# vovach777/llcomp

Hardware: AMD Instinct MI355X
Metric: encode+decode MPix/s on 4K RGB8, bit-exact (higher is better)
Workload: dtype int32

## Files before the change

llcomp_amd/csrc/codec.hip:

```cpp
#include <hip/hip_runtime.h>

#include <algorithm>
#include <cstdlib>
#include <cstring>
#include <mutex>
#include <new>
#include <vector>

#include "../../include/llcomp_mi.h"
#include "codec_internal.hpp"
#include "container.hpp"
#include "geometry.hpp"
#include "kernels.hpp"
#include "resize.hpp"
#include "snapshot.hpp"
#include "tables.hpp"
#include "update.hpp"

using namespace llcomp_mi;

namespace llcomp_mi {

int status_from_bits(uint32_t bits) {
    if (bits & kStInternal) return LLCOMP_MI_HIP_ERROR;
// ... 571 lines not shown
                 uint64_t* d_total, uint32_t* d_status, hipStream_t s) {
    Timed t(k, s, 3);
    if (!encoder_writes_group_sums(g)) HIP_TRY(launch_group_sums(g, d_slice_len, d_group_off, s));
    HIP_TRY(launch_scan_groups(g, d_group_off, d_total, s));
    HIP_TRY(launch_pack_payload(g, k->d_scratch, d_slice_len, d_group_off, d_payload, payload_cap, d_status, s));
    return LLCOMP_MI_OK;
}

}

namespace llcomp_mi {
void codec_release(llcomp_mi_codec* k) {
    if (!k) return;
    DeviceGuard guard(k->device);
    if (k->done && k->done->ev && hipEventQuery(k->done->ev) != hipErrorNotReady) {
        (void)hipGetLastError();
        k->done.reset();
    }
    dev_free(k->d_sym_or_rec, k->done);
    dev_free(k->d_lane_order, k->done);
    dev_free(k->d_states, k->done);
    dev_free(k->d_scratch, k->done);
    dev_free(k->d_group_off, k->done);
    dev_free(k->d_total_tmp, k->done);
    dev_free(k->d_region_len, k->done);
    dev_free(k->d_region_off, k->done);
    dev_free(k->d_regions, k->done);
    dev_free(k->d_stage, k->done);
    dev_free(k->d_box, k->done);
    dev_free(k->d_mid, k->done);
    dev_free(k->d_upd_goff, k->done);
    for (uint32_t i = 0; i < llcomp_mi_codec::kRegionsRing; ++i) {
        if (!k->h_regions[i]) continue;
        if (k->regions_ev_live[i] && k->regions_ev[i] && hipEventQuery(k->regions_ev[i]) == hipErrorNotReady) (void)hipEventSynchronize(k->regions_ev[i]);
        (void)hipGetLastError();
        (void)hipHostFree(k->h_regions[i]);
    }
    for (auto& ev : k->regions_ev) if (ev) (void)hipEventDestroy(ev);
    dev_free(k->d_snap_sorted, k->done);
    dev_free(k->d_snap_banks, k->done);
    dev_free(k->d_snap_res, k->done);
    dev_free(k->d_snap_ctx, k->done);
    dev_free(k->d_snap_io, k->done);
    dev_free(k->d_seg_state, k->done);
    if (k->ev_fork) (void)hipEventDestroy(k->ev_fork);
    for (auto& ev : k->ev_chunk) if (ev) (void)hipEventDestroy(ev);
// ... 74 lines not shown
    if (!guard.ok) return LLCOMP_MI_HIP_ERROR;
    llcomp_mi_codec* k = new (std::nothrow) llcomp_mi_codec;
    if (!k) return LLCOMP_MI_NOMEM;
    k->g = g;
    k->tune = current_tuning();
    k->device = dev;
    k->feedback = !current_tuning().nofeedback;
    k->overlap = current_tuning().overlap != 0;
    k->aux_shared = current_tuning().overlap == 2;
    const uint64_t samples = uint64_t(frames) * w * h * c;
    k->need_states = slices_need_state_tables(g);
    const bool fused = model_is_fused(g);
    const uint64_t b_sym = fused ? 8 : samples * 4, b_states = k->need_states ? (uint64_t(lane_groups(g)) * kContexts << g.lane_shift) * 8 : 8,
                   b_scratch = (uint64_t(lane_groups(g)) << g.lane_shift) * g.slice_cap, b_off = (uint64_t(lane_groups(g)) + 1) * 8;
    const bool snap = snapshot_mode(g);
    const uint64_t snap_el = snap ? snapshot_elems(g) : 0;
    const uint64_t b_lanes = std::max((uint64_t(lane_groups(g)) * slice_capacity_samples(g) << g.lane_shift) * (fused ? 2 : 4), snap_el * 4);
    const uint64_t b_region = uint64_t(g.n_slices) * 12 +
                              (!k->need_states && !rows_mode(g) ? (uint64_t(lane_groups(g)) * kContexts << g.lane_shift) * 8 : 0);
    const uint64_t b_regions = uint64_t(frames) * sizeof(RegionsFrame) + stage_bound(g);
    const uint64_t b_resized = 2 * samples + resized_tables_bound(g);
    const uint64_t b_update = (uint64_t(g.n_slices) + 1 + lane_groups(g) + 1) * 8 +
                              (snap ? 0 : region_snapshot_bound(g) ? region_snapshot_bound(g) * 28 + uint64_t(g.n_slices) * 64 : 0);
    k->workspace_bytes = b_sym + b_lanes + b_states + b_scratch + b_off + 8 + snap_el * (snapshot_chunked(g) ? 28 : 18) + b_region + b_regions +
                         b_resized + b_update;
    const bool ok = dev_alloc(&k->d_sym_or_rec, b_sym) == hipSuccess && dev_alloc(&k->d_lane_order, b_lanes) == hipSuccess &&
                    dev_alloc(reinterpret_cast<void**>(&k->d_scratch), b_scratch) == hipSuccess &&
                    dev_alloc(reinterpret_cast<void**>(&k->d_group_off), b_off) == hipSuccess &&
                    dev_alloc(reinterpret_cast<void**>(&k->d_total_tmp), 8) == hipSuccess &&
                    dev_alloc(reinterpret_cast<void**>(&k->d_counters), kCtrCount * 8) == hipSuccess &&
                    hipMemset(k->d_counters, 0, kCtrCount * 8) == hipSuccess;
    if (!ok) {
        llcomp_mi_codec_destroy(k);
        return LLCOMP_MI_NOMEM;
    }
    k->allocated_bytes = b_sym + b_lanes + b_scratch + b_off + 8;
    *out = k;
    return LLCOMP_MI_OK;
}

extern "C" {

void llcomp_mi_codec_destroy(llcomp_mi_codec* k) {
    llcomp_mi::codec_release(k);
}

int llcomp_mi_codec_prepare(llcomp_mi_codec* k, uint32_t what) {
    if (!k || (what & ~(LLCOMP_MI_PREPARE_ENCODE | LLCOMP_MI_PREPARE_DECODE | LLCOMP_MI_PREPARE_REGION | LLCOMP_MI_PREPARE_REGIONS |
                        LLCOMP_MI_PREPARE_RESIZED | LLCOMP_MI_PREPARE_UPDATE)))
        return LLCOMP_MI_BAD_ARGS;
    DeviceGuard guard(k->device);
    if (!guard.ok) return LLCOMP_MI_HIP_ERROR;
    if (what & LLCOMP_MI_PREPARE_ENCODE) {
        if (snapshot_mode(k->g)) {
            if (int rc = ensure_snapshot_arrays(k, k->g)) return rc;
        }
        if (!snapshot_mode(k->g) || snapshot_chunked(k->g))
            if (int rc = ensure_state_tables(k, k->need_states)) return rc;
    }
// ... 60 lines not shown
    if (!guard.ok) return LLCOMP_MI_HIP_ERROR;
    hipStream_t s = static_cast<hipStream_t>(stream);
    const Geometry& g = k->g;
    DoneGuard done_guard{k, s};
    HIP_TRY(hipMemsetAsync(d_status, 0, 4, s));
    {
        Timed t(k, s, 7);
        if (int rc = next_state_generation(k, s, k->need_states)) return rc;
    }
    {
        Timed t(k, s, 4);
        HIP_TRY(launch_group_sums(g, static_cast<const uint32_t*>(d_slice_len), k->d_group_off, s));
        HIP_TRY(launch_scan_groups(g, k->d_group_off, k->d_total_tmp, s));
    }
    {
        Timed t(k, s, 4);
        HIP_TRY(launch_stage_streams(g, static_cast<const uint8_t*>(d_payload), payload_bytes,
                                     static_cast<const uint32_t*>(d_slice_len), k->d_group_off, k->d_scratch,
                                     static_cast<uint32_t*>(d_status), s));
    }
    {
        Timed t(k, s, 5);
        const bool cache = use_bank_cache(k, g);
        HIP_TRY(launch_decode_slices(g, k->d_scratch, static_cast<const uint32_t*>(d_slice_len), k->d_states, k->state_generation,
                                     static_cast<int16_t*>(k->d_lane_order), static_cast<uint32_t*>(d_status), k->d_counters, cache, s));
        if (cache) queue_feedback(k, s);
    }
    {
        Timed t(k, s, 6);
        if (model_is_fused(g)) {
            HIP_TRY(launch_model_rows_inv(g, static_cast<const int16_t*>(k->d_lane_order), static_cast<uint8_t*>(d_px), s));
        } else {
            HIP_TRY(launch_from_lane_order_i16(g, static_cast<const int16_t*>(k->d_lane_order),
                                               static_cast<int16_t*>(k->d_sym_or_rec), s));
            HIP_TRY(launch_model_inv(g, static_cast<const int16_t*>(k->d_sym_or_rec), static_cast<uint8_t*>(d_px), s));
        }
    }
    ++k->n_decode;
    return LLCOMP_MI_OK;
}

uint32_t llcomp_mi_codec_region_family(const llcomp_mi_codec* k, uint32_t x, uint32_t y, uint32_t rw, uint32_t rh) {
    RegionBox box;
    Geometry sub;
    if (!k || region_setup(k, x, y, rw, rh, box, sub)) return 0;
    return (sub.flags & 0xFFu) | (sub.lane_shift << 8) | (sub.lpw << 16);
}

int llcomp_mi_codec_decode_region(llcomp_mi_codec* k, const void* d_payload, uint64_t payload_bytes, const void* d_slice_len, uint32_t x,
                                  uint32_t y, uint32_t rw, uint32_t rh, void* d_px, void* d_status, void* stream) {
    if (!k || !d_payload || !d_slice_len || !d_px || !d_status) return LLCOMP_MI_BAD_ARGS;
    RegionBox box;
    Geometry sub;
    if (int rc = region_setup(k, x, y, rw, rh, box, sub)) return rc;
// ... 440 lines not shown
```

llcomp_amd/csrc/codec_internal.hpp:

```cpp
#pragma once
#include <hip/hip_runtime.h>

#include <cstdint>
#include <memory>
#include <vector>

#include "../../include/llcomp_mi.h"
#include "geometry.hpp"
#include "kernels.hpp"

namespace llcomp_mi {
struct DoneEvent {
    hipEvent_t ev = nullptr;
    ~DoneEvent();
};
std::shared_ptr<DoneEvent> make_done_event();
}

struct llcomp_mi_codec {
    llcomp_mi::Geometry g{};
    int device = 0;
    void* d_sym_or_rec = nullptr;
    void* d_lane_order = nullptr;
    uint64_t* d_states = nullptr;
    uint8_t* d_scratch = nullptr;
    uint64_t* d_group_off = nullptr;
    uint64_t* d_total_tmp = nullptr;
    uint32_t* d_region_len = nullptr;
    uint64_t* d_region_off = nullptr;
    llcomp_mi::Tuning tune{};
    static constexpr uint32_t kRegionsRing = 4;
    llcomp_mi::RegionsFrame* d_regions = nullptr;
    uint8_t* h_regions[kRegionsRing] = {};
    uint64_t h_regions_cap[kRegionsRing] = {};
    hipEvent_t regions_ev[kRegionsRing] = {};
    bool regions_ev_live[kRegionsRing] = {};
    uint32_t regions_slot = 0;
    uint8_t* d_stage = nullptr;
    uint64_t stage_cap = 0;
    uint8_t* d_box = nullptr;
    uint64_t box_cap = 0;
    uint8_t* d_mid = nullptr;
    uint64_t mid_cap = 0;
    uint64_t* d_upd_goff = nullptr;
    uint64_t snap_el = 0;
    void* d_snap_sorted = nullptr;
    void* d_snap_banks = nullptr;
    void* d_snap_res = nullptr;
    void* d_snap_ctx = nullptr;
    void* d_snap_io = nullptr;
// ... 107 lines not shown
```

llcomp_amd/csrc/geometry.hpp:

```cpp
#pragma once
#include <algorithm>
#include <cstdint>
#include <cstdlib>

#if defined(__HIPCC__)
#define LLMI_HD __host__ __device__
#else
#define LLMI_HD
#endif

namespace llcomp_mi {

constexpr uint32_t kMaxChannels = 255;

struct Geometry {
    uint32_t frames, w, h, c;
    uint32_t tile_w, tile_h, planar;
    uint32_t ntx, nty;
    uint32_t slices_per_frame;
    uint32_t n_slices;
    uint32_t slice_cap;
    uint32_t nch;
    uint32_t lane_shift;
    uint32_t slice_samples;
    uint32_t lpw;
    uint32_t flags;
};
enum : uint32_t {
    kGeoRows = 1u,
    kGeoLdsTable = 2u,
    kGeoForceReplay = 4u,
    kGeoSmallModel = 8u,
    kGeoSnapshot = 16u,
    kGeoBankCache = 32u,
};
constexpr uint32_t kSnapMaxSamples = 4096;
constexpr uint32_t kSnapMaxChunks = 4;

struct Tuning {
    int lane_shift = -1;
    int lpw = 0;
    bool norows = false;
    bool noldstab = false;
    bool force_replay = false;
    bool nosnap = false;
    bool nocache = false;
    int overlap = 2;
    bool nofeedback = false;
};
inline Tuning tuning_from_env() {
    Tuning t;
    auto num = [](const char* name, long lo, long hi, int dflt) {
        const char* e = std::getenv(name);
        if (!e || !*e) return dflt;
        const long v = std::strtol(e, nullptr, 10);
        return (v >= lo && v <= hi) ? int(v) : dflt;
    };
    auto flag = [](const char* name) { const char* e = std::getenv(name); return e && e[0] == '1'; };
    t.lane_shift = num("LLCOMP_MI_LANE_SHIFT", 0, 6, -1);
    t.lpw = num("LLCOMP_MI_LPW", 1, 64, 0);
    t.norows = flag("LLCOMP_MI_NOROWS");
    t.noldstab = flag("LLCOMP_MI_NOLDSTAB");
    t.force_replay = flag("LLCOMP_MI_FORCE_REPLAY");
    t.nosnap = flag("LLCOMP_MI_NOSNAP");
    t.nocache = flag("LLCOMP_MI_NOCACHE");
    t.nofeedback = flag("LLCOMP_MI_NOFEEDBACK");
    t.overlap = num("LLCOMP_MI_OVERLAP", 0, 2, 2);
    return t;
}

LLMI_HD inline uint32_t snapshot_chunks(const Geometry& g) { return (g.slice_samples + kSnapMaxSamples - 1) / kSnapMaxSamples; }
LLMI_HD inline uint32_t snapshot_cap(const Geometry& g) {
    return g.slice_samples <= kSnapMaxSamples ? (g.slice_samples + 15u) & ~15u : snapshot_chunks(g) * kSnapMaxSamples;
}

constexpr int kBankCacheLog2 = 5;
inline int bank_cache_log2(const Geometry& g) { return (g.flags & kGeoBankCache) ? kBankCacheLog2 : 0; }

LLMI_HD inline uint32_t rows_px_dwords(uint64_t tile_base, uint32_t samples, uint32_t c, uint64_t batch_bytes) {
    if (tile_base + 4 > batch_bytes) return 0;
    const uint64_t k = (batch_bytes - 4 - tile_base) / c + 1;
    return k < samples ? uint32_t(k) : samples;
}
LLMI_HD inline uint32_t rows_px_tail(uint32_t c) { return 1 + (4 + c - 1) / c; }

LLMI_HD inline size_t lane_order_index(const Geometry& g, uint32_t id, uint32_t k) {
    const uint32_t gw = 1u << g.lane_shift;
    return ((size_t(id >> g.lane_shift) * g.slice_samples + k) << g.lane_shift) + (id & (gw - 1));
// ... 199 lines not shown
```

llcomp_amd/csrc/kernels.hpp:

```cpp
#pragma once
#include <hip/hip_runtime.h>

#include <cstdint>

#include "geometry.hpp"

namespace llcomp_mi {

enum : uint32_t { kStOverflow = 1u, kStBadExponent = 2u, kStTruncated = 4u, kStInternal = 8u  };

enum : uint32_t {
    kCtrDecCachedWaves = 0,
    kCtrDecBypassedWaves = 1,
    kCtrCacheLookups = 2,
    kCtrCacheMisses = 3,
    kCtrCacheWritebacks = 4,
    kCtrDecReplays = 5,
    kCtrEncCarryBacks = 6,
    kCtrGenerationWraps = 7,
    kCtrDecLaunchesCached = 8,
    kCtrDecLaunchesPlainByFeedback = 9,
    kCtrCount = 16,
};

// ... 16 lines not shown
hipError_t launch_encode_slices(const Geometry& g, const void* d_sym, uint64_t* d_states, uint32_t generation, uint8_t* d_scratch,
                                uint32_t* d_slice_len, uint64_t* d_group_off, uint32_t* d_status, unsigned long long* d_counters,
                                hipStream_t stream);
uint64_t state_generation_tag(uint32_t generation);
hipError_t launch_encode_segment(const Geometry& g, const void* d_res, uint64_t* d_banks, uint8_t* d_scratch, uint32_t* d_slice_len,
                                 uint32_t* d_status, unsigned long long* d_counters, uint32_t seg_first, uint32_t* d_seg_state,
                                 hipStream_t stream);
bool encoder_writes_group_sums(const Geometry& g);
hipError_t launch_group_sums(const Geometry& g, const uint32_t* d_slice_len, uint64_t* d_group_off, hipStream_t stream);
hipError_t launch_scan_groups(const Geometry& g, uint64_t* d_group_off, uint64_t* d_total, hipStream_t stream);
hipError_t launch_frame_bytes(const Geometry& g, const uint32_t* d_slice_len, uint64_t* d_frame_bytes, hipStream_t stream);
hipError_t launch_pack_payload(const Geometry& g, const uint8_t* d_units, const uint32_t* d_slice_len,
                               const uint64_t* d_group_off, uint8_t* d_payload, uint64_t payload_cap,
                               uint32_t* d_status, hipStream_t stream);
hipError_t launch_stage_streams(const Geometry& g, const uint8_t* d_payload, uint64_t payload_bytes,
                                const uint32_t* d_slice_len, const uint64_t* d_group_off, uint8_t* d_units,
                                uint32_t* d_status, hipStream_t stream);
hipError_t launch_copy_segments(const uint8_t* d_src, uint8_t* d_dst, const uint64_t* d_src_off, const uint64_t* d_dst_off,
                                const uint64_t* d_len, uint32_t n_seg, uint64_t max_len, hipStream_t stream);
hipError_t launch_range_sums(const uint32_t* d_vals, const uint64_t* d_start, const uint64_t* d_count, uint64_t* d_out, uint32_t n,
                             uint32_t cap, hipStream_t stream);
hipError_t launch_decode_slices(const Geometry& g, const uint8_t* d_units, const uint32_t* d_slice_len,
                                uint64_t* d_states, uint32_t generation, int16_t* d_rec, uint32_t* d_status, unsigned long long* d_counters,
                                bool bank_cache, hipStream_t stream);

hipError_t launch_region_index(const Geometry& full, const Geometry& sub, const RegionBox& box, const uint32_t* d_slice_len,
                               const uint64_t* d_group_off, uint32_t* d_sub_len, uint64_t* d_sub_off, hipStream_t stream);
hipError_t launch_stage_region_streams(const Geometry& sub, const uint8_t* d_payload, uint64_t payload_bytes, const uint32_t* d_sub_len,
                                       const uint64_t* d_sub_off, uint8_t* d_units, uint32_t* d_status, hipStream_t stream);
struct Crop {
    uint32_t x0, y0, rw, rh;
};
hipError_t launch_model_inv_crop(const Geometry& sub, const int16_t* d_rec, uint8_t* d_px, const Crop& cr, hipStream_t stream);
hipError_t launch_model_rows_inv_crop(const Geometry& sub, const int16_t* d_lanes, uint8_t* d_px, const Crop& cr, hipStream_t stream);

hipError_t launch_regions_index(const Geometry& full, const Geometry& sub, const RegionsFrame* d_tab, const uint32_t* d_slice_len,
                                const uint64_t* d_group_off, uint32_t* d_sub_len, uint64_t* d_sub_off, hipStream_t stream);
hipError_t launch_model_inv_crops(const Geometry& sub, const int16_t* d_rec, uint8_t* d_px, const RegionsFrame* d_tab, uint32_t rw,
                                  uint32_t rh, hipStream_t stream);
hipError_t launch_model_rows_inv_crops(const Geometry& sub, const int16_t* d_lanes, uint8_t* d_px, const RegionsFrame* d_tab, uint32_t rw,
                                       uint32_t rh, hipStream_t stream);

}
```

llcomp_amd/csrc/model_kernels.hip:

```cpp
#include <algorithm>

#include "device_common.hpp"
#include "kernels.hpp"

namespace llcomp_mi {

namespace {

constexpr int kMW = 256;
constexpr int kMH = 32;

template <int C>
__device__ __forceinline__ void rct_forward(const uint8_t* p, int16_t (&o)[C]) {
    if constexpr (C >= 3) {
        const int g = p[1], cb = int(p[2]) - g, cr = int(p[0]) - g;
        o[0] = int16_t(cr);
        o[1] = int16_t(g + (cb + cr) / 4);
        o[2] = int16_t(cb);
        if constexpr (C == 4) o[3] = p[3];
    } else {
#pragma unroll
        for (int k = 0; k < C; ++k) o[k] = p[k];
    }
}

template <int C>
// ... 583 lines not shown
__host__ inline uint64_t xcd_grid(uint32_t n_groups, uint32_t chunks) { return uint64_t((n_groups + kXcds - 1) / kXcds) * kXcds * chunks; }
__device__ __forceinline__ bool xcd_chunk_group(uint32_t n_groups, uint32_t chunks, uint32_t& group, uint32_t& chunk) {
    const uint32_t xcd = blockIdx.x % kXcds, slot = blockIdx.x / kXcds;
    const uint32_t per_class = (chunks + kXcds - 1) / kXcds;
    group = slot / per_class;
    chunk = xcd + kXcds * (slot - group * per_class);
    return group < n_groups && chunk < chunks;
}
__host__ inline uint64_t xcd_chunk_grid(uint32_t n_groups, uint32_t chunks) { return uint64_t(n_groups) * ((chunks + kXcds - 1) / kXcds) * kXcds; }

template <int C>
__device__ __forceinline__ void rct_pixel(const uint8_t* p, int (&v)[C]) {
    if constexpr (C >= 3) {
        const int g = p[1], cb = int(p[2]) - g, cr = int(p[0]) - g;
        v[0] = cr;
        v[1] = g + (cb + cr) / 4;
        v[2] = cb;
        if constexpr (C == 4) v[3] = p[3];
    } else {
#pragma unroll
        for (int k = 0; k < C; ++k) v[k] = p[k];
    }
}
struct RowTile {
    unsigned long long base;
    uint32_t sw;
};
template <int C>
__device__ __forceinline__ void load_row_tiles(const Geometry& g, uint32_t first_tile, uint32_t ntiles, RowTile* tiles) {
    if (threadIdx.x < ntiles) {
        const uint32_t tile = first_tile + threadIdx.x;
        const uint32_t per_frame = g.ntx * g.nty;
        const uint32_t frame = tile / per_frame, rem = tile - frame * per_frame;
        const uint32_t y = rem / g.ntx, tx = rem - y * g.ntx;
        const uint32_t x0 = tx * g.tile_w;
        tiles[threadIdx.x].base = ((size_t(frame) * g.h + y) * g.w + x0) * C;
        tiles[threadIdx.x].sw = g.w - x0 < g.tile_w ? g.w - x0 : g.tile_w;
    }
}

typedef short s16x2 __attribute__((ext_vector_type(2)));
typedef unsigned short u16x2 __attribute__((ext_vector_type(2)));
__device__ __forceinline__ u16x2 pk_min_u16(u16x2 a, u16x2 b) {
    u16x2 d;
    asm("v_pk_min_u16 %0, %1, %2" : "=v"(d) : "v"(a), "v"(b));
    return d;
}

template <int C>
__global__ __launch_bounds__(256) void k_model_rows_fwd(const Geometry g, const uint8_t* __restrict__ px,
                                                        uint16_t* __restrict__ lanes) {
    constexpr int K = 64, RUN = (K + 2) * C, TPG = 64 / C + 2;
    constexpr int RUNW = (RUN + 3) / 4 + 1;
    constexpr int PADL = (C - 1 + 1) & ~1, OCOLS = (PADL + 64 + C - 1 + 1) & ~1;
    __shared__ uint32_t raw[TPG][RUNW + 1];
    __shared__ __attribute__((aligned(4))) uint16_t otile[K][OCOLS];
    __shared__ RowTile tiles[TPG];
    const uint32_t chunks = (g.tile_w + K - 1) / K;
    uint32_t group, chunk;
    if (!xcd_group_chunk((g.n_slices + (1u << g.lane_shift) - 1) >> g.lane_shift, chunks, group, chunk)) return;
    const uint32_t k0 = chunk * K;
    const uint32_t gw = 1u << g.lane_shift;
// ... 143 lines not shown
            *reinterpret_cast<uint32_t*>(&tile[kk][2 * d]) = w[it];
        }
    }
    if (g.lane_shift != 6) {
        __syncthreads();
        for (uint32_t i = threadIdx.x; i < uint32_t(K) * gw; i += 256) {
            const uint32_t kk = i / gw, col = i - kk * gw, k = k0 + kk;
            tile[kk][col] = (first_id + col < g.n_slices && k < g.tile_w) ? lanes[lane_order_index(g, first_id + col, k)] : int16_t(0);
        }
    }
    if constexpr (C > 1) {
        for (uint32_t i = threadIdx.x; i < uint32_t(K) * (C - 1); i += 256) {
            const uint32_t kk = i / (C - 1), e = i - kk * (C - 1), k = k0 + kk;
            const uint32_t id = first_id + gw + e;
            tile[kk][gw + e] = (id < g.n_slices && k < g.tile_w) ? lanes[lane_order_index(g, id, k)] : int16_t(0);
        }
    }
    __syncthreads();
    const uint32_t col0 = first_tile * C - first_id;
    const uint32_t q4 = threadIdx.x & 15;
    for (uint32_t tt = threadIdx.x >> 4; tt < ntiles; tt += 16) {
        const uint32_t sw = tiles[tt].sw, kb = k0 + 4 * q4;
        if (kb >= sw) continue;
        uint8_t bytes[4 * C];
#pragma unroll
        for (int i = 0; i < 4; ++i) {
            const int16_t* s = &tile[4 * q4 + i][col0 + tt * C];
            if constexpr (C >= 3) {
                int r = s[0], gg = s[1], bb = s[2];
                gg -= (r + bb) / 4;
                r += gg;
                bb += gg;
                bytes[i * C + 0] = uint8_t(min(max(r, 0), 255));
                bytes[i * C + 1] = uint8_t(min(max(gg, 0), 255));
                bytes[i * C + 2] = uint8_t(min(max(bb, 0), 255));
                if constexpr (C == 4) bytes[i * C + 3] = uint8_t(s[3]);
            } else {
#pragma unroll
                for (int c = 0; c < C; ++c) bytes[i * C + c] = uint8_t(s[c]);
            }
        }
        uint8_t* o = px + tiles[tt].base + size_t(kb) * C;
        const uint32_t npx = sw - kb < 4 ? sw - kb : 4;
        if (npx == 4) {
            uint32_t w[C];
#pragma unroll
            for (int c = 0; c < C; ++c)
                w[c] = uint32_t(bytes[4 * c]) | (uint32_t(bytes[4 * c + 1]) << 8) | (uint32_t(bytes[4 * c + 2]) << 16) |
                       (uint32_t(bytes[4 * c + 3]) << 24);
            __builtin_memcpy(o, w, 4 * C);
        } else {
            for (uint32_t i = 0; i < npx * C; ++i) o[i] = bytes[i];
        }
    }
}

struct RowTileCrop {
    long long base;
    uint32_t klo, khi;
};
template <int C>
__device__ __forceinline__ void load_row_tiles_crop(const Geometry& g, uint32_t first_tile, uint32_t ntiles, const Crop& cr,
                                                    RowTileCrop* tiles) {
    if (threadIdx.x < ntiles) {
        const uint32_t tile = first_tile + threadIdx.x;
        const uint32_t per_frame = g.ntx * g.nty;
        const uint32_t frame = tile / per_frame, rem = tile - frame * per_frame;
        const uint32_t y = rem / g.ntx, tx = rem - y * g.ntx;
        const uint32_t x0 = tx * g.tile_w;
        const uint32_t sw = g.w - x0 < g.tile_w ? g.w - x0 : g.tile_w;
        const uint32_t klo = cr.x0 > x0 ? cr.x0 - x0 : 0u;
        uint32_t khi = cr.x0 + cr.rw > x0 ? min(sw, cr.x0 + cr.rw - x0) : 0u;
        if (y < cr.y0 || y >= cr.y0 + cr.rh || khi <= klo) khi = 0;
        tiles[threadIdx.x].base = ((long long)(size_t(frame) * cr.rh + (y - cr.y0)) * cr.rw + (long long)x0 - (long long)cr.x0) * C;
        tiles[threadIdx.x].klo = klo;
        tiles[threadIdx.x].khi = khi;
// ... 425 lines not shown
```

llcomp_amd/csrc/slice_kernels.hip:

```cpp
#include <algorithm>

#include "device_common.hpp"
#include "kernels.hpp"

#ifndef LLMI_ASM_ENC
#define LLMI_ASM_ENC 1
#endif
#if LLMI_ASM_ENC
#include "enc_rows_asm.hpp"
#endif
#ifndef LLMI_ASM_DEC
#define LLMI_ASM_DEC 1
#endif
#if LLMI_ASM_DEC
#include "dec_rows_asm.hpp"
#endif

namespace llcomp_mi {

namespace {

#ifdef LLMI_CLOCK_PROBE
constexpr uint32_t kProbeSlots = 1u << 15;
__device__ unsigned long long g_probe[2][kProbeSlots][2];
struct ProbeStamp {
    unsigned long long t, r;
// ... 866 lines not shown
    } else
#endif
    {
        ok = hot ? dec_residual<true, false, INLDS>(d, bank, tab, v) : dec_residual<false, false, INLDS>(d, bank, tab, v);
        hot = 2 * __popcll(__ballot(v != 0)) >= __popcll(__ballot(true));
    }
    const bool ran_dry = (INLDS && LLMI_ASM_DEC != 0) ? false : d.win == 0;
    if (__builtin_expect(!ok || ran_dry || replay_always, 0)) {
        ++d.replays;
        d.low = s_low; d.range = s_range; d.win = s_win;
        bank.w[0] = s_b0; bank.w[1] = s_b1;
        if constexpr (INLDS) {
            bank.w[2] = s_b2; bank.w[3] = s_b3;
            reinterpret_cast<uint32_t*>(bank.lds)[0] = s_b0;
            reinterpret_cast<uint32_t*>(bank.lds)[64] = s_b1;
            reinterpret_cast<uint32_t*>(bank.lds)[128] = s_b2;
            reinterpret_cast<uint32_t*>(bank.lds)[192] = s_b3;
        }
        ok = dec_residual<false, true, INLDS>(d, bank, tab, v);
    }
    return ok;
}

constexpr uint32_t bank_cache_lds_bytes(int log2_entries) { return log2_entries ? (64u * 9u) << log2_entries : 0u; }
template <int NCH, bool ROWS, bool LDSTAB = false, int CACHE = 0>
__global__ __launch_bounds__(64) void k_decode_slices(const Geometry g, const uint32_t lpw_and_flags,
                                                      const uint8_t* __restrict__ units,
                                                      const uint32_t* __restrict__ slice_len,
                                                      uint64_t* __restrict__ states, int16_t* __restrict__ rec,
                                                      uint32_t* status, const uint64_t gpat,
                                                      unsigned long long* __restrict__ counters) {
    __shared__ entry_t tab[128];
    __shared__ uint32_t rowbank[ROWS ? kWideBankWords : 1];
    __shared__ int8_t quant_lut[ROWS ? 1 : 512];
    if constexpr (!ROWS) {
        for (uint32_t i = threadIdx.x; i < 256; i += blockDim.x) {
            quant_lut[i] = int8_t(quant11(int(i) - 128));
            quant_lut[256 + i] = int8_t(quant5(int(i) - 128));
        }
    }
    static_assert(CACHE == 0 || (!ROWS && !LDSTAB && NCH != 0), "the bank cache belongs to the 2-D kernels with tables in HBM");
    static_assert(CACHE == 0 || ((kContexts - 1) >> CACHE) < 0xFF, "bank cache: a context's tag would alias the empty marker");
    __shared__ uint32_t wave_sums[CACHE != 0 ? 2 : 1];
    clear_lds_states<LDSTAB>();
    if constexpr (CACHE != 0) {
        uint32_t* tg = reinterpret_cast<uint32_t*>(dyn_lds + (512u << CACHE));
        for (uint32_t i = threadIdx.x; i < (16u << CACHE); i += blockDim.x) tg[i] = 0xFFFFFFFFu;
        if (threadIdx.x < 2) wave_sums[threadIdx.x] = 0;
    }
    load_table(tab);
    const uint32_t lpw = lpw_and_flags & 0xFF;
    const bool replay_always = (lpw_and_flags >> 8) & 1;
    const bool small_model = (g.flags & kGeoSmallModel) != 0;
    const uint32_t id = blockIdx.x * lpw + threadIdx.x;
    if (threadIdx.x >= lpw || id >= g.n_slices) return;
    const SliceRect r = slice_rect(g, id);
    RangeDec d;
    const uint32_t len = min(slice_len[id], g.slice_cap - 16);
    const uint32_t grp = __builtin_amdgcn_readfirstlane(id >> g.lane_shift);
    const uint32_t lane_in_group = id & ((1u << g.lane_shift) - 1);
    dec_open(d, reinterpret_cast<const uint32_t*>(units) + ((size_t(grp) * (g.slice_cap >> 2)) << g.lane_shift), lane_in_group,
             g.lane_shift, len);

    int16_t* p0 = rec + lane_order_index(g, id, 0);
    const ptrdiff_t GW = ptrdiff_t(1) << g.lane_shift;
    int16_t* const gbase = rec + ((size_t(grp) * g.slice_samples) << g.lane_shift);
    uint32_t hot = 0;
    LLMI_PROBE_START();

    if constexpr (ROWS) {
        for (uint32_t k = 0; k < 12; ++k) rowbank[k * 64 + threadIdx.x] = lds_address(tab) * 0x00010001u;
        int l[NCH], L[NCH];
#pragma unroll
        for (int k = 0; k < NCH; ++k) l[k] = L[k] = 128;
        int held_val = 0;
        uint32_t held_ofs = lane_in_group * 2, next_ofs = held_ofs, step_ofs = 2u << g.lane_shift;
        uint32_t large = small_model ? 0u : ~0u, first = ~0u;
        asm volatile("" : "+v"(large), "+v"(first), "+v"(step_ofs));
        uint8_t* const bank0 = reinterpret_cast<uint8_t*>(rowbank) + threadIdx.x * 4;
        bool bad = false;
        auto pixel = [&]() {
// ... 10 lines not shown
                asm volatile("" : "+v"(o1), "+v"(o2));
                uint32_t* bp = reinterpret_cast<uint32_t*>(bank0 + (o1 + o2));
                Bank bank{{bp[0], bp[64], bp[128], bp[192]}, reinterpret_cast<uint8_t*>(bp)};
                uint32_t v = 0;
                if (!dec_sample<true>(d, bank, tab, hot, replay_always, v)) bad = true;
                v = (v ^ uint32_t(sg)) - uint32_t(sg);
                const int val = int(int16_t(uint32_t(lv) + v));
                held_val = val;
                held_ofs = next_ofs;
                next_ofs += step_ofs;
                L[k] = lv ^ ((lv ^ val) & int(first));
                l[k] = val;
            }
            first = 0;
        };
        const uint32_t sw0 = __builtin_amdgcn_readfirstlane(r.sw);
        const uint32_t n_bulk = __builtin_amdgcn_ballot_w64(r.sw != sw0) == 0 ? sw0 : 0;
        uint32_t x = 0;
        for (; x < n_bulk; ++x) pixel();
        for (; x < r.sw; ++x) pixel();
        if (bad) atomicOr(status, kStBadExponent);
        asm volatile("global_store_short %0, %1, %2" : : "v"(held_ofs), "v"(held_val), "s"(gbase) : "memory");
        publish_count(counters, kCtrDecReplays, d.replays);
    } else {
        uint64_t* banks;
        uint32_t bsh;
        if constexpr (LDSTAB) {
            banks = reinterpret_cast<uint64_t*>(dyn_lds);
            bsh = 0;
        } else {
            banks = states + ((size_t(id >> g.lane_shift) * kContexts) << g.lane_shift) + (id & ((1u << g.lane_shift) - 1));
            bsh = g.lane_shift;
        }
        if constexpr (NCH == 0) {
            const uint32_t nch = g.nch;
            const ptrdiff_t px_step = ptrdiff_t(nch) * GW, up = ptrdiff_t(r.sw) * px_step;
            for (uint32_t y = 0; y < r.sh; ++y) {
                for (uint32_t x = 0; x < r.sw; ++x) {
                    for (uint32_t k = 0; k < nch; ++k) {
                        int16_t* q = p0 + ptrdiff_t(y) * up + ptrdiff_t(x) * px_step + ptrdiff_t(k) * GW;
                        if (window_low(d)) dec_append(d);
                        const Hood n = apply_borders(x > 0 ? q[-px_step] : 0, x > 1 ? q[-2 * px_step] : 0, y > 0 ? q[-up] : 0,
                                                     (y > 0 && x > 0) ? q[-up - px_step] : 0, (y > 0 && x + 1 < r.sw) ? q[-up + px_step] : 0,
                                                     y > 1 ? q[-2 * up] : 0, x, y, r.sw);
                        int ctx = context_hash(n, small_model);
                        const bool neg = ctx < 0;
// ... 184 lines not shown
        case 9: { constexpr int C = 2; constexpr bool R = false; constexpr bool T = true; __VA_ARGS__; } break;     \
        case 10: { constexpr int C = 2; constexpr bool R = true; constexpr bool T = false; __VA_ARGS__; } break;    \
        case 12: { constexpr int C = 3; constexpr bool R = false; constexpr bool T = false; __VA_ARGS__; } break;   \
        case 13: { constexpr int C = 3; constexpr bool R = false; constexpr bool T = true; __VA_ARGS__; } break;    \
        case 14: { constexpr int C = 3; constexpr bool R = true; constexpr bool T = false; __VA_ARGS__; } break;    \
        case 16: { constexpr int C = 4; constexpr bool R = false; constexpr bool T = false; __VA_ARGS__; } break;   \
        case 17: { constexpr int C = 4; constexpr bool R = false; constexpr bool T = true; __VA_ARGS__; } break;    \
        case 18: { constexpr int C = 4; constexpr bool R = true; constexpr bool T = false; __VA_ARGS__; } break;    \
        default: return hipErrorInvalidValue;                                                               \
    }

bool rows_mode(const Geometry& g) { return (g.flags & kGeoRows) != 0; }
static bool states_in_lds(const Geometry& g) { return (g.flags & kGeoLdsTable) != 0; }
bool slices_need_state_tables(const Geometry& g) { return !rows_mode(g) && !states_in_lds(g); }

constexpr size_t kLdsTableBytes = size_t(kContexts) * 8;
template <typename K>
hipError_t allow_big_lds(K kernel) {
    return hipFuncSetAttribute(reinterpret_cast<const void*>(kernel), hipFuncAttributeMaxDynamicSharedMemorySize,
                               int(kLdsTableBytes));
}

static bool coder_in_segments(const Geometry& g) { return (g.flags & kGeoSnapshot) != 0 && snapshot_chunks(g) > 1; }
bool encoder_writes_group_sums(const Geometry& g) { return g.lpw == (1u << g.lane_shift) && !coder_in_segments(g); }

hipError_t launch_encode_segment(const Geometry& g, const void* d_res, uint64_t* d_banks, uint8_t* d_scratch, uint32_t* d_slice_len,
                                 uint32_t* d_status, unsigned long long* d_counters, uint32_t seg_first, uint32_t* d_seg_state,
                                 hipStream_t stream) {
    if (!coder_in_segments(g) || !d_seg_state) return hipErrorInvalidValue;
    const uint32_t blocks = (g.n_slices + g.lpw - 1) / g.lpw;
    k_encode_slices<0, false, uint32_t, false, true, true><<<dim3(blocks), dim3(64), LLMI_ASM_ENC ? kRowsEncLdsBytes : 0, stream>>>(
        g, g.lpw, static_cast<const uint32_t*>(d_res), d_banks, d_scratch, d_slice_len, nullptr, d_status, 0, d_counters, seg_first, d_seg_state);
    return hipGetLastError();
}

uint64_t state_generation_tag(uint32_t generation) {
    uint64_t t = 0;
    for (int i = 0; i < 8; ++i) t |= uint64_t((generation >> i) & 1u) << (8 * i + 7);
    return t;
}

hipError_t launch_encode_slices(const Geometry& g, const void* d_sym, uint64_t* d_states, uint32_t generation, uint8_t* d_scratch,
                                uint32_t* d_slice_len, uint64_t* d_group_off, uint32_t* d_status, unsigned long long* d_counters,
                                hipStream_t stream) {
    const uint64_t gpat = slices_need_state_tables(g) ? state_generation_tag(generation) : 0;
    const uint32_t lpw = g.lpw;
// ... 9 lines not shown
            g, lpw, static_cast<const uint16_t*>(d_sym), d_states, d_scratch, d_slice_len, d_group_sum, d_status, gpat, d_counters);
        return hipGetLastError();
    }
    if (g.flags & kGeoSnapshot) {
        k_encode_slices<0, false, uint32_t, false, true><<<dim3(blocks), dim3(64), LLMI_ASM_ENC ? kRowsEncLdsBytes : 0, stream>>>(
            g, lpw, static_cast<const uint32_t*>(d_sym), d_states, d_scratch, d_slice_len, d_group_sum, d_status, 0, d_counters);
        return hipGetLastError();
    }
    const bool lds = states_in_lds(g);
    LLMI_DISPATCH_SLICE(g.nch, rows_mode(g), lds, {
        auto kernel = k_encode_slices<C, R, uint32_t, T>;
        if (T) {
            const hipError_t e = allow_big_lds(kernel);
            if (e != hipSuccess) return e;
        }
        kernel<<<dim3(blocks), dim3(64), T ? kLdsTableBytes : (R && LLMI_ASM_ENC ? kRowsEncLdsBytes : 0), stream>>>(
            g, lpw, static_cast<const uint32_t*>(d_sym), d_states, d_scratch, d_slice_len, d_group_sum, d_status, gpat, d_counters, 0u, nullptr);
    });
    return hipGetLastError();
}

hipError_t launch_decode_slices(const Geometry& g, const uint8_t* d_units, const uint32_t* d_slice_len,
                                uint64_t* d_states, uint32_t generation, int16_t* d_rec, uint32_t* d_status, unsigned long long* d_counters,
                                bool bank_cache, hipStream_t stream) {
    const uint64_t gpat = slices_need_state_tables(g) ? state_generation_tag(generation) : 0;
    const uint32_t lpw = g.lpw;
    const uint32_t blocks = (g.n_slices + lpw - 1) / lpw;
    const uint32_t arg = lpw | ((g.flags & kGeoForceReplay) ? 0x100u : 0u);
    const bool lds = states_in_lds(g);
    if (bank_cache_log2(g) == kBankCacheLog2 && bank_cache) {
#define LLMI_DECODE_CACHED(NCHV)                                                                                          \
    k_decode_slices<NCHV, false, false, kBankCacheLog2><<<dim3(blocks), dim3(64), bank_cache_lds_bytes(kBankCacheLog2), stream>>>( \
        g, arg, d_units, d_slice_len, d_states, d_rec, d_status, gpat, d_counters)
        switch (g.nch) {
            case 1: LLMI_DECODE_CACHED(1); break;
            case 2: LLMI_DECODE_CACHED(2); break;
            case 3: LLMI_DECODE_CACHED(3); break;
            case 4: LLMI_DECODE_CACHED(4); break;
            default: return hipErrorInvalidValue;
        }
#undef LLMI_DECODE_CACHED
        return hipGetLastError();
    }
    LLMI_DISPATCH_SLICE(g.nch, rows_mode(g), lds, {
        auto kernel = k_decode_slices<C, R, T>;
        if (T) {
            const hipError_t e = allow_big_lds(kernel);
            if (e != hipSuccess) return e;
        }
        kernel<<<dim3(blocks), dim3(64), T ? kLdsTableBytes : 0, stream>>>(g, arg, d_units, d_slice_len, d_states,
                                                                          d_rec, d_status, gpat, d_counters);
    });
    return hipGetLastError();
}

}
```

Before: 29020.

## Fuse inverse color model into rows decoder epilogue with ticketed straddling tiles

When the fused rows model runs with 64-lane groups, the decode kernel now performs the inverse color transform and writes pixels itself. This removes the separate launch_model_rows_inv kernel and its extra round trip through the lane-order buffer. For 3 channels, tiles that straddle two workgroups are handled by per-group atomic tickets, so whichever group finishes second writes the shared tile. The cost is a memset per decode, extra LDS reuse of the row banks, and added epilogue work and synchronisation inside an already latency-bound decoder.

```diff
diff --git a/llcomp_amd/csrc/codec.hip b/llcomp_amd/csrc/codec.hip
--- a/llcomp_amd/csrc/codec.hip
+++ b/llcomp_amd/csrc/codec.hip
@@ -617,6 +617,7 @@
     dev_free(k->d_states, k->done);
     dev_free(k->d_scratch, k->done);
     dev_free(k->d_group_off, k->done);
+    dev_free(k->d_inv_tickets, k->done);
     dev_free(k->d_total_tmp, k->done);
     dev_free(k->d_region_len, k->done);
     dev_free(k->d_region_off, k->done);
@@ -737,19 +738,22 @@
     const uint64_t b_resized = 2 * samples + resized_tables_bound(g);
     const uint64_t b_update = (uint64_t(g.n_slices) + 1 + lane_groups(g) + 1) * 8 +
                               (snap ? 0 : region_snapshot_bound(g) ? region_snapshot_bound(g) * 28 + uint64_t(g.n_slices) * 64 : 0);
-    k->workspace_bytes = b_sym + b_lanes + b_states + b_scratch + b_off + 8 + snap_el * (snapshot_chunked(g) ? 28 : 18) + b_region + b_regions +
+    k->fused_inv = rows_decoder_writes_pixels(g) && !k->tune.nofusedinv;
+    const uint64_t b_tickets = k->fused_inv ? rows_decoder_ticket_bytes(g) : 0;
+    k->workspace_bytes = b_tickets + b_sym + b_lanes + b_states + b_scratch + b_off + 8 + snap_el * (snapshot_chunked(g) ? 28 : 18) + b_region + b_regions +
                          b_resized + b_update;
     const bool ok = dev_alloc(&k->d_sym_or_rec, b_sym) == hipSuccess && dev_alloc(&k->d_lane_order, b_lanes) == hipSuccess &&
                     dev_alloc(reinterpret_cast<void**>(&k->d_scratch), b_scratch) == hipSuccess &&
                     dev_alloc(reinterpret_cast<void**>(&k->d_group_off), b_off) == hipSuccess &&
                     dev_alloc(reinterpret_cast<void**>(&k->d_total_tmp), 8) == hipSuccess &&
+                    (b_tickets == 0 || dev_alloc(reinterpret_cast<void**>(&k->d_inv_tickets), b_tickets) == hipSuccess) &&
                     dev_alloc(reinterpret_cast<void**>(&k->d_counters), kCtrCount * 8) == hipSuccess &&
                     hipMemset(k->d_counters, 0, kCtrCount * 8) == hipSuccess;
     if (!ok) {
         llcomp_mi_codec_destroy(k);
         return LLCOMP_MI_NOMEM;
     }
-    k->allocated_bytes = b_sym + b_lanes + b_scratch + b_off + 8;
+    k->allocated_bytes = b_sym + b_lanes + b_scratch + b_off + 8 + b_tickets;
     *out = k;
     return LLCOMP_MI_OK;
 }
@@ -856,14 +860,16 @@
     {
         Timed t(k, s, 5);
         const bool cache = use_bank_cache(k, g);
+        if (k->d_inv_tickets) HIP_TRY(hipMemsetAsync(k->d_inv_tickets, 0, rows_decoder_ticket_bytes(g), s));
         HIP_TRY(launch_decode_slices(g, k->d_scratch, static_cast<const uint32_t*>(d_slice_len), k->d_states, k->state_generation,
-                                     static_cast<int16_t*>(k->d_lane_order), static_cast<uint32_t*>(d_status), k->d_counters, cache, s));
+                                     static_cast<int16_t*>(k->d_lane_order), static_cast<uint32_t*>(d_status), k->d_counters, cache, s,
+                                     k->fused_inv ? static_cast<uint8_t*>(d_px) : nullptr, k->d_inv_tickets));
         if (cache) queue_feedback(k, s);
     }
     {
         Timed t(k, s, 6);
         if (model_is_fused(g)) {
-            HIP_TRY(launch_model_rows_inv(g, static_cast<const int16_t*>(k->d_lane_order), static_cast<uint8_t*>(d_px), s));
+            if (!k->fused_inv) HIP_TRY(launch_model_rows_inv(g, static_cast<const int16_t*>(k->d_lane_order), static_cast<uint8_t*>(d_px), s));
         } else {
             HIP_TRY(launch_from_lane_order_i16(g, static_cast<const int16_t*>(k->d_lane_order),
                                                static_cast<int16_t*>(k->d_sym_or_rec), s));
diff --git a/llcomp_amd/csrc/codec_internal.hpp b/llcomp_amd/csrc/codec_internal.hpp
--- a/llcomp_amd/csrc/codec_internal.hpp
+++ b/llcomp_amd/csrc/codec_internal.hpp
@@ -26,6 +26,8 @@
     uint8_t* d_scratch = nullptr;
     uint64_t* d_group_off = nullptr;
     uint64_t* d_total_tmp = nullptr;
+    bool fused_inv = false;
+    uint32_t* d_inv_tickets = nullptr;
     uint32_t* d_region_len = nullptr;
     uint64_t* d_region_off = nullptr;
     llcomp_mi::Tuning tune{};
diff --git a/llcomp_amd/csrc/geometry.hpp b/llcomp_amd/csrc/geometry.hpp
--- a/llcomp_amd/csrc/geometry.hpp
+++ b/llcomp_amd/csrc/geometry.hpp
@@ -46,6 +46,7 @@
     bool nosnap = false;
     bool nocache = false;
     int overlap = 2;
+    bool nofusedinv = false;
     bool nofeedback = false;
 };
 inline Tuning tuning_from_env() {
@@ -64,6 +65,7 @@
     t.force_replay = flag("LLCOMP_MI_FORCE_REPLAY");
     t.nosnap = flag("LLCOMP_MI_NOSNAP");
     t.nocache = flag("LLCOMP_MI_NOCACHE");
+    t.nofusedinv = flag("LLCOMP_MI_NOFUSEDINV");
     t.nofeedback = flag("LLCOMP_MI_NOFEEDBACK");
     t.overlap = num("LLCOMP_MI_OVERLAP", 0, 2, 2);
     return t;
diff --git a/llcomp_amd/csrc/kernels.hpp b/llcomp_amd/csrc/kernels.hpp
--- a/llcomp_amd/csrc/kernels.hpp
+++ b/llcomp_amd/csrc/kernels.hpp
@@ -62,7 +62,9 @@
                              uint32_t cap, hipStream_t stream);
 hipError_t launch_decode_slices(const Geometry& g, const uint8_t* d_units, const uint32_t* d_slice_len,
                                 uint64_t* d_states, uint32_t generation, int16_t* d_rec, uint32_t* d_status, unsigned long long* d_counters,
-                                bool bank_cache, hipStream_t stream);
+                                bool bank_cache, hipStream_t stream, uint8_t* d_px = nullptr, uint32_t* d_tickets = nullptr);
+bool rows_decoder_writes_pixels(const Geometry& g);
+uint64_t rows_decoder_ticket_bytes(const Geometry& g);
 
 hipError_t launch_region_index(const Geometry& full, const Geometry& sub, const RegionBox& box, const uint32_t* d_slice_len,
                                const uint64_t* d_group_off, uint32_t* d_sub_len, uint64_t* d_sub_off, hipStream_t stream);
diff --git a/llcomp_amd/csrc/model_kernels.hip b/llcomp_amd/csrc/model_kernels.hip
--- a/llcomp_amd/csrc/model_kernels.hip
+++ b/llcomp_amd/csrc/model_kernels.hip
@@ -2,6 +2,7 @@
 
 #include "device_common.hpp"
 #include "kernels.hpp"
+#include "rows_model.hpp"
 
 namespace llcomp_mi {
 
@@ -631,22 +632,6 @@
         for (int k = 0; k < C; ++k) v[k] = p[k];
     }
 }
-struct RowTile {
-    unsigned long long base;
-    uint32_t sw;
-};
-template <int C>
-__device__ __forceinline__ void load_row_tiles(const Geometry& g, uint32_t first_tile, uint32_t ntiles, RowTile* tiles) {
-    if (threadIdx.x < ntiles) {
-        const uint32_t tile = first_tile + threadIdx.x;
-        const uint32_t per_frame = g.ntx * g.nty;
-        const uint32_t frame = tile / per_frame, rem = tile - frame * per_frame;
-        const uint32_t y = rem / g.ntx, tx = rem - y * g.ntx;
-        const uint32_t x0 = tx * g.tile_w;
-        tiles[threadIdx.x].base = ((size_t(frame) * g.h + y) * g.w + x0) * C;
-        tiles[threadIdx.x].sw = g.w - x0 < g.tile_w ? g.w - x0 : g.tile_w;
-    }
-}
 
 typedef short s16x2 __attribute__((ext_vector_type(2)));
 typedef unsigned short u16x2 __attribute__((ext_vector_type(2)));
@@ -836,36 +821,8 @@
     for (uint32_t tt = threadIdx.x >> 4; tt < ntiles; tt += 16) {
         const uint32_t sw = tiles[tt].sw, kb = k0 + 4 * q4;
         if (kb >= sw) continue;
-        uint8_t bytes[4 * C];
-#pragma unroll
-        for (int i = 0; i < 4; ++i) {
-            const int16_t* s = &tile[4 * q4 + i][col0 + tt * C];
-            if constexpr (C >= 3) {
-                int r = s[0], gg = s[1], bb = s[2];
-                gg -= (r + bb) / 4;
-                r += gg;
-                bb += gg;
-                bytes[i * C + 0] = uint8_t(min(max(r, 0), 255));
-                bytes[i * C + 1] = uint8_t(min(max(gg, 0), 255));
-                bytes[i * C + 2] = uint8_t(min(max(bb, 0), 255));
-                if constexpr (C == 4) bytes[i * C + 3] = uint8_t(s[3]);
-            } else {
-#pragma unroll
-                for (int c = 0; c < C; ++c) bytes[i * C + c] = uint8_t(s[c]);
-            }
-        }
-        uint8_t* o = px + tiles[tt].base + size_t(kb) * C;
-        const uint32_t npx = sw - kb < 4 ? sw - kb : 4;
-        if (npx == 4) {
-            uint32_t w[C];
-#pragma unroll
-            for (int c = 0; c < C; ++c)
-                w[c] = uint32_t(bytes[4 * c]) | (uint32_t(bytes[4 * c + 1]) << 8) | (uint32_t(bytes[4 * c + 2]) << 16) |
-                       (uint32_t(bytes[4 * c + 3]) << 24);
-            __builtin_memcpy(o, w, 4 * C);
-        } else {
-            for (uint32_t i = 0; i < npx * C; ++i) o[i] = bytes[i];
-        }
+        rows_inv_store<C>([&](int i) { return &tile[4 * q4 + i][col0 + tt * C]; }, px + tiles[tt].base + size_t(kb) * C,
+                          sw - kb < 4 ? sw - kb : 4);
     }
 }
 
diff --git a/llcomp_amd/csrc/rows_model.hpp b/llcomp_amd/csrc/rows_model.hpp
--- /dev/null
+++ b/llcomp_amd/csrc/rows_model.hpp
@@ -0,0 +1,62 @@
+#pragma once
+#include <hip/hip_runtime.h>
+
+#include <cstdint>
+
+#include "geometry.hpp"
+
+namespace llcomp_mi {
+
+struct RowTile {
+    unsigned long long base;
+    uint32_t sw;
+};
+template <int C>
+__device__ __forceinline__ RowTile row_tile(const Geometry& g, uint32_t tile) {
+    const uint32_t per_frame = g.ntx * g.nty;
+    const uint32_t frame = tile / per_frame, rem = tile - frame * per_frame;
+    const uint32_t y = rem / g.ntx, tx = rem - y * g.ntx;
+    const uint32_t x0 = tx * g.tile_w;
+    RowTile t;
+    t.base = ((size_t(frame) * g.h + y) * g.w + x0) * C;
+    t.sw = g.w - x0 < g.tile_w ? g.w - x0 : g.tile_w;
+    return t;
+}
+template <int C>
+__device__ __forceinline__ void load_row_tiles(const Geometry& g, uint32_t first_tile, uint32_t ntiles, RowTile* tiles) {
+    if (threadIdx.x < ntiles) tiles[threadIdx.x] = row_tile<C>(g, first_tile + threadIdx.x);
+}
+
+template <int C, typename S>
+__device__ __forceinline__ void rows_inv_store(S sample, uint8_t* o, uint32_t npx) {
+    uint8_t bytes[4 * C];
+#pragma unroll
+    for (int i = 0; i < 4; ++i) {
+        const int16_t* s = sample(i);
+        if constexpr (C >= 3) {
+            int r = s[0], gg = s[1], bb = s[2];
+            gg -= (r + bb) / 4;
+            r += gg;
+            bb += gg;
+            bytes[i * C + 0] = uint8_t(min(max(r, 0), 255));
+            bytes[i * C + 1] = uint8_t(min(max(gg, 0), 255));
+            bytes[i * C + 2] = uint8_t(min(max(bb, 0), 255));
+            if constexpr (C == 4) bytes[i * C + 3] = uint8_t(s[3]);
+        } else {
+#pragma unroll
+            for (int c = 0; c < C; ++c) bytes[i * C + c] = uint8_t(s[c]);
+        }
+    }
+    if (npx == 4) {
+        uint32_t w[C];
+#pragma unroll
+        for (int c = 0; c < C; ++c)
+            w[c] = uint32_t(bytes[4 * c]) | (uint32_t(bytes[4 * c + 1]) << 8) | (uint32_t(bytes[4 * c + 2]) << 16) |
+                   (uint32_t(bytes[4 * c + 3]) << 24);
+        __builtin_memcpy(o, w, 4 * C);
+    } else {
+        for (uint32_t i = 0; i < npx * C; ++i) o[i] = bytes[i];
+    }
+}
+
+}
diff --git a/llcomp_amd/csrc/slice_kernels.hip b/llcomp_amd/csrc/slice_kernels.hip
--- a/llcomp_amd/csrc/slice_kernels.hip
+++ b/llcomp_amd/csrc/slice_kernels.hip
@@ -2,6 +2,7 @@
 
 #include "device_common.hpp"
 #include "kernels.hpp"
+#include "rows_model.hpp"
 
 #ifndef LLMI_ASM_ENC
 #define LLMI_ASM_ENC 1
@@ -914,14 +915,103 @@
     return ok;
 }
 
+constexpr int kInvChunk = 16;
+constexpr int kInvRow = 64 + 2;
+constexpr uint32_t kInvTileBytes = kInvChunk * kInvRow * 2;
+static_assert(kInvTileBytes % 8 == 0 && kInvTileBytes + 64 * (8 + 4) <= kWideBankWords * 4, "the epilogue lives in the row banks' LDS");
+
+template <int C>
+__device__ __forceinline__ void rows_inv_straddling_tile(const Geometry& g, const int16_t* rec, uint8_t* px, uint32_t tile) {
+    const RowTile t = row_tile<C>(g, tile);
+    for (uint32_t kb = 4 * threadIdx.x; kb < t.sw; kb += 4 * 64) {
+        int16_t v[4][C];
+#pragma unroll
+        for (int i = 0; i < 4; ++i) {
+            const uint32_t k = kb + i < t.sw ? kb + i : t.sw - 1;
+#pragma unroll
+            for (int c = 0; c < C; ++c) v[i][c] = rec[lane_order_index(g, tile * C + c, k)];
+        }
+        rows_inv_store<C>([&](int i) { return &v[i][0]; }, px + t.base + size_t(kb) * C, t.sw - kb < 4 ? t.sw - kb : 4);
+    }
+}
+
+template <int C>
+__device__ __forceinline__ void rows_inv_epilogue(const Geometry& g, uint32_t grp, const int16_t* rec, uint8_t* px, uint32_t* tickets,
+                                                  uint32_t* lds) {
+    const uint32_t lane = threadIdx.x;
+    const uint32_t first_id = grp << 6, end_id = first_id + 64 < g.n_slices ? first_id + 64 : g.n_slices;
+    asm volatile("s_waitcnt vmcnt(0)" ::: "memory");
+    if constexpr (C == 3) {
+        const uint32_t lrem = first_id % 3, rrem = end_id % 3;
+        if (lrem | rrem) {
+            __builtin_amdgcn_fence(__ATOMIC_RELEASE, "agent");
+            asm volatile("s_waitcnt vmcnt(0)" ::: "memory");
+            uint32_t second = 0;
+            if (lane == 0) {
+                if (lrem) second = __hip_atomic_fetch_add(tickets + grp - 1, 1u, __ATOMIC_RELAXED, __HIP_MEMORY_SCOPE_AGENT);
+                if (rrem) second |= __hip_atomic_fetch_add(tickets + grp, 1u, __ATOMIC_RELAXED, __HIP_MEMORY_SCOPE_AGENT) << 1;
+            }
+            second = __builtin_amdgcn_readfirstlane(second);
+            __builtin_amdgcn_fence(__ATOMIC_ACQUIRE, "agent");
+            if (second & 1) rows_inv_straddling_tile<C>(g, rec, px, first_id / 3);
+            if (second & 2) rows_inv_straddling_tile<C>(g, rec, px, end_id / 3);
+        }
+    }
+    const uint32_t first_tile = (first_id + C - 1) / C, end_tile = end_id / C;
+    if (end_tile <= first_tile) return;
+    const uint32_t ntiles = end_tile - first_tile;
+    int16_t (*tile)[kInvRow] = reinterpret_cast<int16_t (*)[kInvRow]>(lds);
+    unsigned long long* t_base = reinterpret_cast<unsigned long long*>(reinterpret_cast<uint8_t*>(lds) + kInvTileBytes);
+    uint32_t* t_sw = reinterpret_cast<uint32_t*>(t_base + 64);
+    if (lane < ntiles) {
+        const RowTile t = row_tile<C>(g, first_tile + lane);
+        t_base[lane] = t.base;
+        t_sw[lane] = t.sw;
+    }
+    const uint32_t n = g.slice_samples, d = lane & 31, half = lane >> 5;
+    const uint32_t* rows = reinterpret_cast<const uint32_t*>(rec + ((size_t(grp) * n) << 6));
+    auto fetch = [&](uint32_t k0, uint32_t (&w)[kInvChunk / 2]) {
+#pragma unroll
+        for (int it = 0; it < kInvChunk / 2; ++it) {
+            const uint32_t k = k0 + 2 * it + half;
+            w[it] = rows[size_t(k < n ? k : n - 1) * 32 + d];
+        }
+    };
+    const uint32_t col0 = first_tile * C - first_id;
+    auto pass = [&](uint32_t k0, const uint32_t (&w)[kInvChunk / 2]) {
+        __syncthreads();
+#pragma unroll
+        for (int it = 0; it < kInvChunk / 2; ++it) *reinterpret_cast<uint32_t*>(&tile[2 * it + half][2 * d]) = w[it];
+        __syncthreads();
+        for (uint32_t i = lane; i < ntiles * (kInvChunk / 4); i += 64) {
+            const uint32_t tt = i / (kInvChunk / 4), q4 = i % (kInvChunk / 4), kb = k0 + 4 * q4, sw = t_sw[tt];
+            if (kb >= sw) continue;
+            const int16_t* s0 = &tile[4 * q4][col0 + tt * C];
+            rows_inv_store<C>([&](int j) { return s0 + j * kInvRow; }, px + t_base[tt] + size_t(kb) * C, sw - kb < 4 ? sw - kb : 4);
+        }
+    };
+    uint32_t wa[kInvChunk / 2], wb[kInvChunk / 2];
+    fetch(0, wa);
+    for (uint32_t k0 = 0;; k0 += 2 * kInvChunk) {
+        fetch(k0 + kInvChunk, wb);
+        pass(k0, wa);
+        if (k0 + kInvChunk >= n) break;
+        fetch(k0 + 2 * kInvChunk, wa);
+        pass(k0 + kInvChunk, wb);
+        if (k0 + 2 * kInvChunk >= n) break;
+    }
+}
+
 constexpr uint32_t bank_cache_lds_bytes(int log2_entries) { return log2_entries ? (64u * 9u) << log2_entries : 0u; }
-template <int NCH, bool ROWS, bool LDSTAB = false, int CACHE = 0>
+template <int NCH, bool ROWS, bool LDSTAB = false, int CACHE = 0, int PXC = 0>
 __global__ __launch_bounds__(64) void k_decode_slices(const Geometry g, const uint32_t lpw_and_flags,
                                                       const uint8_t* __restrict__ units,
                                                       const uint32_t* __restrict__ slice_len,
                                                       uint64_t* __restrict__ states, int16_t* __restrict__ rec,
                                                       uint32_t* status, const uint64_t gpat,
-                                                      unsigned long long* __restrict__ counters) {
+                                                      unsigned long long* __restrict__ counters, uint8_t* __restrict__ px = nullptr,
+                                                      uint32_t* tickets = nullptr) {
+    static_assert(PXC == 0 || (ROWS && NCH == 1 && !LDSTAB && CACHE == 0), "the pixel epilogue belongs to the planar 1-row kernel");
     __shared__ entry_t tab[128];
     __shared__ uint32_t rowbank[ROWS ? kWideBankWords : 1];
     __shared__ int8_t quant_lut[ROWS ? 1 : 512];
@@ -945,10 +1035,16 @@
     const bool replay_always = (lpw_and_flags >> 8) & 1;
     const bool small_model = (g.flags & kGeoSmallModel) != 0;
     const uint32_t id = blockIdx.x * lpw + threadIdx.x;
-    if (threadIdx.x >= lpw || id >= g.n_slices) return;
-    const SliceRect r = slice_rect(g, id);
+    const bool live = PXC == 0 || id < g.n_slices;
+    if constexpr (PXC == 0) {
+        if (threadIdx.x >= lpw || id >= g.n_slices) return;
+    }
+    SliceRect r = slice_rect(g, id);
+    if constexpr (PXC != 0) {
+        if (!live) r.sw = 0;
+    }
     RangeDec d;
-    const uint32_t len = min(slice_len[id], g.slice_cap - 16);
+    const uint32_t len = live ? min(slice_len[id], g.slice_cap - 16) : 0u;
     const uint32_t grp = __builtin_amdgcn_readfirstlane(id >> g.lane_shift);
     const uint32_t lane_in_group = id & ((1u << g.lane_shift) - 1);
     dec_open(d, reinterpret_cast<const uint32_t*>(units) + ((size_t(grp) * (g.slice_cap >> 2)) << g.lane_shift), lane_in_group,
@@ -1005,6 +1101,7 @@
         if (bad) atomicOr(status, kStBadExponent);
         asm volatile("global_store_short %0, %1, %2" : : "v"(held_ofs), "v"(held_val), "s"(gbase) : "memory");
         publish_count(counters, kCtrDecReplays, d.replays);
+        if constexpr (PXC != 0) rows_inv_epilogue<PXC>(g, grp, rec, px, tickets, rowbank);
     } else {
         uint64_t* banks;
         uint32_t bsh;
@@ -1235,6 +1332,10 @@
 }
 
 static bool coder_in_segments(const Geometry& g) { return (g.flags & kGeoSnapshot) != 0 && snapshot_chunks(g) > 1; }
+bool rows_decoder_writes_pixels(const Geometry& g) { return model_is_fused(g) && g.lane_shift == 6 && g.lpw == 64; }
+uint64_t rows_decoder_ticket_bytes(const Geometry& g) {
+    return rows_decoder_writes_pixels(g) && g.c == 3 ? (uint64_t(lane_groups(g)) * 4 + 15) & ~15ull : 0;
+}
 bool encoder_writes_group_sums(const Geometry& g) { return g.lpw == (1u << g.lane_shift) && !coder_in_segments(g); }
 
 hipError_t launch_encode_segment(const Geometry& g, const void* d_res, uint64_t* d_banks, uint8_t* d_scratch, uint32_t* d_slice_len,
@@ -1290,12 +1391,27 @@
 
 hipError_t launch_decode_slices(const Geometry& g, const uint8_t* d_units, const uint32_t* d_slice_len,
                                 uint64_t* d_states, uint32_t generation, int16_t* d_rec, uint32_t* d_status, unsigned long long* d_counters,
-                                bool bank_cache, hipStream_t stream) {
+                                bool bank_cache, hipStream_t stream, uint8_t* d_px, uint32_t* d_tickets) {
     const uint64_t gpat = slices_need_state_tables(g) ? state_generation_tag(generation) : 0;
     const uint32_t lpw = g.lpw;
     const uint32_t blocks = (g.n_slices + lpw - 1) / lpw;
     const uint32_t arg = lpw | ((g.flags & kGeoForceReplay) ? 0x100u : 0u);
     const bool lds = states_in_lds(g);
+    if (d_px) {
+        if (!rows_decoder_writes_pixels(g) || (g.c == 3 && !d_tickets)) return hipErrorInvalidValue;
+#define LLMI_DECODE_PX(CV)                                                                                                          \
+    k_decode_slices<1, true, false, 0, CV><<<dim3(blocks), dim3(64), 0, stream>>>(g, arg, d_units, d_slice_len, d_states, d_rec, d_status, \
+                                                                                  gpat, d_counters, d_px, d_tickets)
+        switch (g.c) {
+            case 1: LLMI_DECODE_PX(1); break;
+            case 2: LLMI_DECODE_PX(2); break;
+            case 3: LLMI_DECODE_PX(3); break;
+            case 4: LLMI_DECODE_PX(4); break;
+            default: return hipErrorInvalidValue;
+        }
+#undef LLMI_DECODE_PX
+        return hipGetLastError();
+    }
     if (bank_cache_log2(g) == kBankCacheLog2 && bank_cache) {
 #define LLMI_DECODE_CACHED(NCHV)                                                                                          \
     k_decode_slices<NCHV, false, false, kBankCacheLog2><<<dim3(blocks), dim3(64), bank_cache_lds_bytes(kBankCacheLog2), stream>>>( \
@@ -1317,7 +1433,7 @@
             if (e != hipSuccess) return e;
         }
         kernel<<<dim3(blocks), dim3(64), T ? kLdsTableBytes : 0, stream>>>(g, arg, d_units, d_slice_len, d_states,
-                                                                          d_rec, d_status, gpat, d_counters);
+                                                                          d_rec, d_status, gpat, d_counters, nullptr, nullptr);
     });
     return hipGetLastError();
 }
```

New measurement: 26940. -7.2%, worse.
